# HumanCompatibleAI/overcooked_ai

Measured on NVIDIA H100. Metric: env-steps/sec (joint transitions), higher is better.
Workload: dtype int32

## Files before the change

### overcooked_ai_b200/csrc/ovc_b200.cu

```cuda
#include <cuda.h>
#include <cuda_runtime.h>
#include <stdint.h>
#include <stdio.h>
#include <stdlib.h>
#include <string.h>

#include "../../include/ovc_b200.h"
#include "ovc_step.cuh"

namespace ovc {

static thread_local char g_err[512] = "";

static int fail(int code, const char *msg) {
    snprintf(g_err, sizeof g_err, "%s", msg);
    return code;
}
static int fail(int code, const char *msg, long long value) {
    snprintf(g_err, sizeof g_err, "%s (got %lld)", msg, value);
    return code;
}
static int cuda_fail(cudaError_t e, const char *what) {
    snprintf(g_err, sizeof g_err, "%s: %s", what, cudaGetErrorString(e));
    return OVC_E_CUDA;
}

__device__ __forceinline__ uint32_t smem_u32(const void *p) { return (uint32_t)__cvta_generic_to_shared(p); }

__device__ __forceinline__ void mbar_init(uint64_t *bar, int count) {
    asm volatile("mbarrier.init.shared::cta.b64 [%0], %1;" ::"r"(smem_u32(bar)), "r"(count) : "memory");
    asm volatile("fence.mbarrier_init.release.cluster;" ::: "memory");
    asm volatile("fence.proxy.async.shared::cta;" ::: "memory");
}
__device__ __forceinline__ void mbar_expect_tx(uint64_t *bar, uint32_t bytes) {
    asm volatile("mbarrier.arrive.expect_tx.shared::cta.b64 _, [%0], %1;" ::"r"(smem_u32(bar)), "r"(bytes) : "memory");
}
__device__ __forceinline__ void mbar_wait(uint64_t *bar, uint32_t parity) {
    uint32_t ok;
    do {
        asm volatile(
            "{\n\t.reg .pred p;\n\t"
            "mbarrier.try_wait.parity.shared::cta.b64 p, [%1], %2;\n\t"
            "selp.u32 %0, 1, 0, p;\n\t}"
            : "=r"(ok)
            : "r"(smem_u32(bar)), "r"(parity)
            : "memory");
    } while (!ok);
}
__device__ __forceinline__ void fence_async_smem() { asm volatile("fence.proxy.async.shared::cta;" ::: "memory"); }

__device__ __forceinline__ void tma_load_2d(void *dst, const CUtensorMap *map, int c0, int c1, uint64_t *bar) {
    asm volatile(
        "cp.async.bulk.tensor.2d.shared::cluster.global.tile.mbarrier::complete_tx::bytes [%0], [%1, {%2, %3}], [%4];"
        ::"r"(smem_u32(dst)), "l"((uint64_t)map), "r"(c0), "r"(c1), "r"(smem_u32(bar))
        : "memory");
}
__device__ __forceinline__ void tma_store_2d(const CUtensorMap *map, int c0, int c1, const void *src) {
    asm volatile("cp.async.bulk.tensor.2d.global.shared::cta.tile.bulk_group [%0, {%1, %2}], [%3];" ::"l"((uint64_t)map),
                 "r"(c0), "r"(c1), "r"(smem_u32(src))
                 : "memory");
}
__device__ __forceinline__ void prefetch_tmap(const CUtensorMap *map) {
    asm volatile("prefetch.tensormap [%0];" ::"l"((uint64_t)map) : "memory");
}
__device__ __forceinline__ void prefetch_l2(const void *p) { asm volatile("prefetch.global.L2 [%0];" ::"l"(p)); }
__device__ __forceinline__ void bulk_load_1d(void *dst, const void *src, uint32_t bytes, uint64_t *bar) {
    asm volatile("cp.async.bulk.shared::cluster.global.mbarrier::complete_tx::bytes [%0], [%1], %2, [%3];" ::"r"(
                     smem_u32(dst)),
                 "l"((uint64_t)src), "r"(bytes), "r"(smem_u32(bar))
                 : "memory");
}
__device__ __forceinline__ void bulk_store_1d(void *dst, const void *src, uint32_t bytes) {
    asm volatile("cp.async.bulk.global.shared::cta.bulk_group [%0], [%1], %2;" ::"l"((uint64_t)dst), "r"(smem_u32(src)),
                 "r"(bytes)
                 : "memory");
}
__device__ __forceinline__ void bulk_commit() { asm volatile("cp.async.bulk.commit_group;" ::: "memory"); }
template <int N>
__device__ __forceinline__ void bulk_wait_read() {
    asm volatile("cp.async.bulk.wait_group.read %0;" ::"n"(N) : "memory");
}

template <int S, int SWZ>
struct SmemRec {
    char *tile;
    uint32_t base;
    __device__ __forceinline__ uint32_t phys(uint32_t off) const {
        if (SWZ == 0) return off;
        return off ^ (((off >> 7) & ((1u << SWZ) - 1u)) << 4);
    }
    __device__ __forceinline__ int4 ld4(int c) const { return *reinterpret_cast<const int4 *>(tile + phys(base + c * 16)); }
    __device__ __forceinline__ void st4(int c, int4 v) { *reinterpret_cast<int4 *>(tile + phys(base + c * 16)) = v; }
    __device__ __forceinline__ int ldw(int w) const { return *reinterpret_cast<const int *>(tile + phys(base + w * 4)); }
    __device__ __forceinline__ void stw(int w, int v) { *reinterpret_cast<int *>(tile + phys(base + w * 4)) = v; }
};

struct GlobalRec {
    int32_t *rec;
    __device__ __forceinline__ int4 ld4(int c) const { return *reinterpret_cast<const int4 *>(rec + c * 4); }
    __device__ __forceinline__ void st4(int c, int4 v) { *reinterpret_cast<int4 *>(rec + c * 4) = v; }
    __device__ __forceinline__ int ldw(int w) const { return rec[w]; }
    __device__ __forceinline__ void stw(int w, int v) { rec[w] = v; }
};

#ifndef OVC_TILE16
#define OVC_TILE16 128
#endif

template <int S>
struct Cfg {
    static constexpr int TILE = S <= 16 ? OVC_TILE16 : S <= 32 ? 128 : 64;
    static constexpr int ROW_WORDS = S == 16 ? 16 : 32;
    static constexpr int ROWS_PER_ENV = S / ROW_WORDS;
    static constexpr int BOX_ROWS = TILE * ROWS_PER_ENV;
    static constexpr int SWZ = S == 16 ? 2 : 3;
    static constexpr int TILE_BYTES = TILE * S * 4;
};

struct StepArgs {
    const ovc_layout_t *layouts;
    const int32_t *start_records;
    int32_t *state;
    const int32_t *actions;
    int32_t *sparse, *shaped, *done, *events;
    long long n_envs;
    int n_layouts;
    int n_steps;
    int horizon, flags;
    int has_rs;
    ovc_random_start_t rs;
};

__host__ __device__ __forceinline__ unsigned delivery_rank(unsigned row) { return (unsigned)((0x0008007605432100ull >> (row * 4)) & 15u); }
__host__ __device__ __forceinline__ unsigned delivery_row(unsigned rank) { return (unsigned)((0xC98654321ull >> (rank * 4)) & 15u); }

__device__ __forceinline__ unsigned event_code(unsigned ev) {
    if ((ev & 0x1FFFFFFu) == 0) return 0;
    if (ev & (1u << OVC_EV_SOUP_DELIVERY)) return 23u + delivery_rank((ev >> OVC_EV_RECIPE_SHIFT) & 15u);
    if (ev & ((1u << OVC_EV_POTTING_ONION) | (1u << OVC_EV_POTTING_TOMATO))) {
        const unsigned tom = (ev >> OVC_EV_POTTING_TOMATO) & 1u;
        const unsigned viable = (ev >> (OVC_EV_VIABLE_ONION_POTTING + tom)) & 1u, optimal = (ev >> (OVC_EV_OPTIMAL_ONION_POTTING + tom)) & 1u;
        const unsigned cata = (ev >> (OVC_EV_CATASTROPHIC_ONION_POTTING + tom)) & 1u;
        return 15u + tom * 4u + (viable ? (optimal ? 0u : 1u) : (cata ? 2u : 3u));
    }
    if (ev & (1u << OVC_EV_SOUP_PICKUP)) return 7;
    if (ev & (1u << OVC_EV_SOUP_DROP)) return 14;
    if (ev & (1u << OVC_EV_ONION_PICKUP)) return 1u + ((ev >> OVC_EV_USEFUL_ONION_PICKUP) & 1u);
    if (ev & (1u << OVC_EV_TOMATO_PICKUP)) return 3u + ((ev >> OVC_EV_USEFUL_TOMATO_PICKUP) & 1u);
    if (ev & (1u << OVC_EV_DISH_PICKUP)) return 5u + ((ev >> OVC_EV_USEFUL_DISH_PICKUP) & 1u);
    if (ev & (1u << OVC_EV_ONION_DROP)) return 8u + ((ev >> OVC_EV_USEFUL_ONION_DROP) & 1u);
    if (ev & (1u << OVC_EV_TOMATO_DROP)) return 10u + ((ev >> OVC_EV_USEFUL_TOMATO_DROP) & 1u);
    return 12u + ((ev >> OVC_EV_USEFUL_DISH_DROP) & 1u);
}

__device__ __forceinline__ unsigned code_word(unsigned c0, unsigned c1, unsigned done, bool stepped, bool grant0, bool grant1) {
    return c0 | (c1 << 5) | (done << 10) | (stepped ? 1u << 11 : 0u) | (grant0 ? 1u << 12 : 0u) | (grant1 ? 1u << 13 : 0u);
}

template <bool WIDE>
__device__ __forceinline__ void write_outputs(const StepArgs &a, long long idx, const StepOut &o) {
    if (!WIDE && (a.flags & OVC_F_OUT_CODES)) {
        reinterpret_cast<unsigned short *>(a.events)[idx] = (unsigned short)code_word(
            event_code(o.ev0), event_code(o.ev1), (unsigned)o.done, o.ev0 & OVC_EVF_STEPPED_DONE, o.shaped0 != 0, o.shaped1 != 0);
        return;
    }
    if (!WIDE && (a.flags & OVC_F_OUT_PACKED)) {
        reinterpret_cast<short *>(a.sparse)[idx] = (short)o.sparse;
        reinterpret_cast<char2 *>(a.shaped)[idx] = make_char2((signed char)o.shaped0, (signed char)o.shaped1);
        reinterpret_cast<unsigned short *>(a.events)[idx] = (unsigned short)code_word(
            event_code(o.ev0), event_code(o.ev1), (unsigned)o.done, o.ev0 & OVC_EVF_STEPPED_DONE, false, false);
        return;
    }
    if (!WIDE && (a.flags & OVC_F_OUT_NARROW)) {
        reinterpret_cast<short *>(a.sparse)[idx] = (short)o.sparse;
        reinterpret_cast<unsigned char *>(a.done)[idx] = (unsigned char)o.done;
        reinterpret_cast<char2 *>(a.shaped)[idx] = make_char2((signed char)o.shaped0, (signed char)o.shaped1);
    } else {
        a.sparse[idx] = o.sparse;
        a.done[idx] = o.done;
        reinterpret_cast<int2 *>(a.shaped)[idx] = make_int2(o.shaped0, o.shaped1);
    }
    reinterpret_cast<int2 *>(a.events)[idx] = make_int2((int)o.ev0, (int)o.ev1);
}

template <bool WIDE, typename I>
__device__ __forceinline__ const void *action_addr(const StepArgs &a, I idx) {
    if (!WIDE && (a.flags & OVC_F_ACT_PACKED)) return reinterpret_cast<const unsigned char *>(a.actions) + idx;
    if (!WIDE && (a.flags & OVC_F_ACT_U8)) return reinterpret_cast<const uchar2 *>(a.actions) + idx;
    return reinterpret_cast<const int2 *>(a.actions) + idx;
}

template <bool WIDE, typename I>
__device__ __forceinline__ int2 load_action(const StepArgs &a, I idx) {
    if (!WIDE && (a.flags & OVC_F_ACT_PACKED)) {
        const unsigned u = *static_cast<const unsigned char *>(action_addr<WIDE>(a, idx));
        return make_int2((int)(u & 15u), (int)(u >> 4));
    }
    if (!WIDE && (a.flags & OVC_F_ACT_U8)) {
        const uchar2 u = *static_cast<const uchar2 *>(action_addr<WIDE>(a, idx));
        return make_int2(u.x, u.y);
    }
    return *static_cast<const int2 *>(action_addr<WIDE>(a, idx));
}

constexpr int MAX_SMEM_LAYOUTS = 8;

template <int S, int IO, bool RS, bool WIDE>
__global__ void __launch_bounds__(Cfg<S>::TILE)
step_kernel(const __grid_constant__ CUtensorMap tmap, const StepArgs a) {
    using C = Cfg<S>;
    const long long env0 = (long long)blockIdx.x * C::TILE;
    const long long env = env0 + threadIdx.x;
    const bool live = env < a.n_envs;
    const int T = a.n_steps;

    if (IO == 3) {
        asm volatile("griddepcontrol.launch_dependents;" ::: "memory");
        asm volatile("griddepcontrol.wait;" ::: "memory");
        if (!live) return;
        GlobalRec r{a.state + env * S};
        const TblG tb{reinterpret_cast<const char *>(a.layouts)};
        for (int t = 0; t < T; t++) {
            const long long idx = (long long)t * a.n_envs + env;
            const int2 act = load_action<WIDE>(a, idx);
            StepOut o;
            step_core<RS>(r, tb, a.start_records, S, act.x, act.y, a.horizon, a.flags, RS ? &a.rs : nullptr, env, a.n_layouts, o);
            write_outputs<WIDE>(a, idx, o);
        }
        return;
    }

    extern __shared__ __align__(1024) char smem[];
    char *tile = smem;
    const int n_tbl = a.n_layouts <= MAX_SMEM_LAYOUTS ? a.n_layouts : 0;
    const uint32_t tbl_bytes = (uint32_t)n_tbl * (uint32_t)sizeof(ovc_layout_t);
    char *tbl = smem + C::TILE_BYTES;
    uint64_t *bar = reinterpret_cast<uint64_t *>(smem + C::TILE_BYTES + tbl_bytes);
    const long long rem = a.n_envs - env0;
    const uint32_t live_bytes = (uint32_t)((rem < C::TILE ? rem : C::TILE) * S * 4);

    if (threadIdx.x == 0) {
        mbar_init(bar, 1);
        mbar_expect_tx(bar, (IO == 1 ? (uint32_t)C::TILE_BYTES : live_bytes) + tbl_bytes);
        if (IO == 1) prefetch_tmap(&tmap);
        if (n_tbl) bulk_load_1d(tbl, a.layouts, tbl_bytes, bar);
    }
    asm volatile("griddepcontrol.wait;" ::: "memory");
    if (threadIdx.x == 0) {
        if (IO == 1) tma_load_2d(tile, &tmap, 0, (int)(env0 * C::ROWS_PER_ENV), bar);
        else bulk_load_1d(tile, a.state + env0 * S, live_bytes, bar);
    }
    int2 act = make_int2(OVC_A_STAY, OVC_A_STAY);
    if (live) act = load_action<WIDE>(a, env);
    __syncthreads();
    mbar_wait(bar, 0);
    asm volatile("griddepcontrol.launch_dependents;" ::: "memory");

    if (live) {
        SmemRec<S, IO == 1 ? C::SWZ : 0> r{tile, (uint32_t)threadIdx.x * S * 4};
        auto run = [&](auto tb) {
            for (int t = 0; t < T; t++) {
                const long long idx = (long long)t * a.n_envs + env;
                int2 nxt = act;
                if (t + 1 < T) nxt = load_action<WIDE>(a, idx + a.n_envs);
                StepOut o;
                step_core<RS>(r, tb, a.start_records, S, act.x, act.y, a.horizon, a.flags, RS ? &a.rs : nullptr, env, a.n_layouts, o);
                write_outputs<WIDE>(a, idx, o);
                act = nxt;
            }
        };
        if (n_tbl) run(TblS{tbl});
        else run(TblG{reinterpret_cast<const char *>(a.layouts)});
    }
    fence_async_smem();
    __syncthreads();
    if (threadIdx.x == 0) {
        if (IO == 1) tma_store_2d(&tmap, 0, (int)(env0 * C::ROWS_PER_ENV), tile);
        else bulk_store_1d(a.state + env0 * S, tile, live_bytes);
        bulk_commit();
        bulk_wait_read<0>();
    }
}

}

#include "ovc_rollout.cuh"

namespace ovc {

__global__ void reset_kernel(const int32_t *__restrict__ start_records, int n_layouts, int32_t *__restrict__ state,
                             const int32_t *__restrict__ env_layout, const int32_t *__restrict__ mask,
                             long long n_envs, int S) {
    const int cpr = S / 4;
    const long long i = (long long)blockIdx.x * blockDim.x + threadIdx.x;
    if (i >= n_envs * cpr) return;
    const long long env = i / cpr;
    const int c = (int)(i % cpr);
    if (mask && mask[env] == 0) return;
    int lid = env_layout ? env_layout[env] : (state[env * S + 3] & 0xFF);
    if (lid < 0 || lid >= n_layouts) lid = 0;
    reinterpret_cast<int4 *>(state)[i] = __ldg(reinterpret_cast<const int4 *>(start_records) + (long long)lid * cpr + c);
}

__global__ void reset_random_kernel(const ovc_layout_t *__restrict__ layouts, int n_layouts,
                                    const int32_t *__restrict__ start_records, int32_t *__restrict__ state,
                                    const int32_t *__restrict__ env_layout, const int32_t *__restrict__ mask,
                                    long long n_envs, int S, const ovc_random_start_t rs) {
    const long long env = (long long)blockIdx.x * blockDim.x + threadIdx.x;
    if (env >= n_envs) return;
    if (mask && mask[env] == 0) return;
    int32_t *rec = state + env * S;
    const unsigned old = (unsigned)rec[3];
    int lid = env_layout ? env_layout[env] : (int)(old & 0xFF);
    const unsigned episode = ((old >> 16) + 1u) & 0xFFFFu;
    if (rs.random_layout) lid = random_layout_id(rs, (uint64_t)env, episode, n_layouts);
    if (lid < 0 || lid >= n_layouts) lid = 0;
    const ovc_layout_t *L = layouts + lid;
    random_start_record([&](int w, int32_t v) { rec[w] = v; }, S, start_records + (size_t)lid * S, L->cook_time, L->free_pos,
                        L->n_free, L->n_pots, lid, rs, (uint64_t)env, episode);
}

typedef CUresult (*encode_tiled_fn)(CUtensorMap *, CUtensorMapDataType, cuuint32_t, void *, const cuuint64_t *,
                                    const cuuint64_t *, const cuuint32_t *, const cuuint32_t *, CUtensorMapInterleave,
                                    CUtensorMapSwizzle, CUtensorMapL2promotion, CUtensorMapFloatOOBfill);

static encode_tiled_fn get_encode_fn() {
    static encode_tiled_fn fn = nullptr;
    static bool tried = false;
    if (!tried) {
        tried = true;
        void *p = nullptr;
        cudaDriverEntryPointQueryResult q;
        if (cudaGetDriverEntryPoint("cuTensorMapEncodeTiled", &p, cudaEnableDefault, &q) == cudaSuccess &&
            q == cudaDriverEntryPointSuccess)
            fn = (encode_tiled_fn)p;
    }
    return fn;
}

template <int S>
static int make_tmap(CUtensorMap *m, int32_t *state, long long n_envs, int box_rows = Cfg<S>::BOX_ROWS) {
    using C = Cfg<S>;
    encode_tiled_fn enc = get_encode_fn();
    if (!enc) return fail(OVC_E_CUDA, "cuTensorMapEncodeTiled entry point not available");
    cuuint64_t dims[2] = {(cuuint64_t)C::ROW_WORDS, (cuuint64_t)(n_envs * C::ROWS_PER_ENV)};
    cuuint64_t strides[1] = {(cuuint64_t)C::ROW_WORDS * 4};
    cuuint32_t box[2] = {(cuuint32_t)C::ROW_WORDS, (cuuint32_t)box_rows};
    cuuint32_t estr[2] = {1, 1};
    CUresult r = enc(m, CU_TENSOR_MAP_DATA_TYPE_INT32, 2, state, dims, strides, box, estr, CU_TENSOR_MAP_INTERLEAVE_NONE,
                     S == 16 ? CU_TENSOR_MAP_SWIZZLE_64B : CU_TENSOR_MAP_SWIZZLE_128B, CU_TENSOR_MAP_L2_PROMOTION_NONE,
                     CU_TENSOR_MAP_FLOAT_OOB_FILL_NONE);
    if (r != CUDA_SUCCESS) return fail(OVC_E_CUDA, "cuTensorMapEncodeTiled failed", (long long)r);
    return OVC_OK;
}

struct OutFmt {
    int act, sparse, shaped, done, events;
    bool stream;
    bool missing(const void *act_p, const void *sparse_p, const void *shaped_p, const void *done_p, const void *events_p) const {
        return !act_p || !events_p || (sparse && !sparse_p) || (shaped && !shaped_p) || (done && !stream && !done_p);
    }
    bool wide() const { return act == 8 && sparse == 4; }
};

static OutFmt formats_of(int flags) {
    OutFmt f;
    f.act = (flags & OVC_F_ACT_PACKED) ? 1 : (flags & OVC_F_ACT_U8) ? 2 : 8;
    f.stream = flags & OVC_F_OUT_STREAM;
    if (f.stream) f.sparse = 2, f.shaped = 0, f.done = 2, f.events = 4;
    else if (flags & OVC_F_OUT_CODES) f.sparse = 0, f.shaped = 0, f.done = 0, f.events = 2;
    else if (flags & OVC_F_OUT_PACKED) f.sparse = 2, f.shaped = 2, f.done = 0, f.events = 2;
    else if (flags & OVC_F_OUT_NARROW) f.sparse = 2, f.shaped = 2, f.done = 1, f.events = 8;
    else f.sparse = 4, f.shaped = 8, f.done = 4, f.events = 8;
    return f;
}

template <int S, int IO>
static cudaError_t launch_one(const CUtensorMap &tmap, const StepArgs &a, unsigned grid, size_t smem, cudaStream_t st) {
    using C = Cfg<S>;
    cudaLaunchConfig_t cfg;
    memset(&cfg, 0, sizeof cfg);
    cfg.gridDim = dim3(grid), cfg.blockDim = dim3(C::TILE), cfg.dynamicSmemBytes = smem, cfg.stream = st;
    cudaLaunchAttribute attr[1];
    attr[0].id = cudaLaunchAttributeProgrammaticStreamSerialization;
    attr[0].val.programmaticStreamSerializationAllowed = 1;
    cfg.attrs = attr;
    cfg.numAttrs = (a.flags & OVC_F_PDL) ? 1 : 0;
    const bool wide = formats_of(a.flags).wide();
    if (a.has_rs)
        return wide ? cudaLaunchKernelEx(&cfg, step_kernel<S, IO, true, true>, tmap, a)
                    : cudaLaunchKernelEx(&cfg, step_kernel<S, IO, true, false>, tmap, a);
    return wide ? cudaLaunchKernelEx(&cfg, step_kernel<S, IO, false, true>, tmap, a)
                : cudaLaunchKernelEx(&cfg, step_kernel<S, IO, false, false>, tmap, a);
}

template <int S, int TILE>
static int launch_rollout(const StepArgs &a, cudaStream_t st) {
    using C = RollCfg<S, TILE>;
    CUtensorMap tmap;
    memset(&tmap, 0, sizeof tmap);
    int rc = make_tmap<S>(&tmap, a.state, a.n_envs, C::BOX_ROWS);
    if (rc) return rc;
    const size_t smem = C::smem_bytes(a.n_layouts);
    const OutFmt f = formats_of(a.flags);
    const bool wide = f.wide(), stream = f.stream;
    void (*kern)(const CUtensorMap, const StepArgs) =
        a.has_rs ? (wide ? rollout_kernel<S, TILE, true, FMT_WIDE> : stream ? rollout_kernel<S, TILE, true, FMT_STREAM> : rollout_kernel<S, TILE, true, FMT_HOST>)
                 : (wide ? rollout_kernel<S, TILE, false, FMT_WIDE> : stream ? rollout_kernel<S, TILE, false, FMT_STREAM> : rollout_kernel<S, TILE, false, FMT_HOST>);
    if (smem > 48 * 1024) {
        cudaError_t e = cudaFuncSetAttribute(kern, cudaFuncAttributeMaxDynamicSharedMemorySize, (int)smem);
        if (e != cudaSuccess) return cuda_fail(e, "rollout kernel shared-memory attribute");
    }
    const long long grid = (a.n_envs + TILE - 1) / TILE;
    StepArgs ka = a;
    ka.flags &= ~F_K5_NO_PREFETCH;
#if OVC_K5_PREFETCH > 1
    {
        int dev = 0, n_sm = 0, per_sm = 0;
        cudaError_t e = cudaGetDevice(&dev);
        if (e == cudaSuccess) e = cudaDeviceGetAttribute(&n_sm, cudaDevAttrMultiProcessorCount, dev);
        if (e == cudaSuccess) e = cudaOccupancyMaxActiveBlocksPerMultiprocessor(&per_sm, kern, TILE, smem);
        if (e != cudaSuccess) return cuda_fail(e, "rollout kernel occupancy");
        const long long warps = grid * (TILE / 32);
        if (grid <= (long long)per_sm * n_sm && (warps >= 24LL * n_sm || warps < 12LL * n_sm)) ka.flags |= F_K5_NO_PREFETCH;
    }
#endif
    cudaLaunchConfig_t cfg;
    memset(&cfg, 0, sizeof cfg);
    cfg.gridDim = dim3((unsigned)grid), cfg.blockDim = dim3(TILE), cfg.dynamicSmemBytes = smem, cfg.stream = st;
    cudaLaunchAttribute attr[1];
    attr[0].id = cudaLaunchAttributeProgrammaticStreamSerialization;
    attr[0].val.programmaticStreamSerializationAllowed = 1;
    cfg.attrs = attr;
    cfg.numAttrs = 0;
    cudaError_t e = cudaLaunchKernelEx(&cfg, kern, tmap, ka);
    if (e != cudaSuccess) return cuda_fail(e, "rollout kernel launch");
    return OVC_OK;
}

static int rollout_tile(int S, long long n_envs, int n_layouts) {
    static int forced = -1;
    if (forced < 0) {
        const char *e = getenv("OVC_K5_TILE");
        forced = e ? atoi(e) : 0;
    }
    (void)n_envs;
    if (S > 32) return 64;
    if (forced == 32 || forced == 64 || forced == 128) return forced;
    return n_layouts >= 3 ? 128 : 64;
}

static bool use_rollout_kernel(const StepArgs &a, int io) {
    static int off = -1;
    if (off < 0) {
        const char *e = getenv("OVC_K5_LEGACY");
        off = e && atoi(e) ? 1 : 0;
    }
    const bool stream = a.flags & OVC_F_OUT_STREAM;
    return (!off || stream) && (a.n_steps > 1 || stream) && a.n_steps <= ROLLOUT_MAX_STEPS && io == 1 && a.n_layouts <= MAX_SMEM_LAYOUTS;
}

template <int S>
static int launch_rollout_tiled(const StepArgs &a, cudaStream_t st) {
    if constexpr (S > 32) {
        return launch_rollout<S, 64>(a, st);
    } else {
        switch (rollout_tile(S, a.n_envs, a.n_layouts)) {
        case 32: return launch_rollout<S, 32>(a, st);
        case 64: return launch_rollout<S, 64>(a, st);
        default: return launch_rollout<S, 128>(a, st);
        }
    }
}

template <int S>
static int launch_rollout_any(const StepArgs &a0, cudaStream_t st) {
    long long max_steps = 0xFFFFFFFFLL / a0.n_envs - 1;
    {
        static long long cap = -1;
        if (cap < 0) {
            const char *e = getenv("OVC_K5_MAX_LAUNCH_STEPS");
            cap = e ? atoll(e) : 0;
        }
        if (cap > 0 && cap < max_steps && !(a0.flags & OVC_F_OUT_STREAM)) max_steps = cap;
    }
    if (a0.n_steps <= max_steps) return launch_rollout_tiled<S>(a0, st);
    if (max_steps < 1 || (a0.flags & OVC_F_OUT_STREAM)) return fail(OVC_E_UNSUPPORTED, "rollout too large for one launch (n_steps * n_envs must stay below 2^32)");
    const OutFmt f = formats_of(a0.flags);
    for (long long t0 = 0; t0 < a0.n_steps; t0 += max_steps) {
        StepArgs a = a0;
        const long long off = t0 * a0.n_envs;
        a.n_steps = (int)(a0.n_steps - t0 < max_steps ? a0.n_steps - t0 : max_steps);
        a.actions = reinterpret_cast<const int32_t *>(reinterpret_cast<const char *>(a0.actions) + off * f.act);
        if (a0.sparse) a.sparse = reinterpret_cast<int32_t *>(reinterpret_cast<char *>(a0.sparse) + off * f.sparse);
        if (a0.shaped) a.shaped = reinterpret_cast<int32_t *>(reinterpret_cast<char *>(a0.shaped) + off * f.shaped);
        if (a0.done) a.done = reinterpret_cast<int32_t *>(reinterpret_cast<char *>(a0.done) + off * f.done);
        a.events = reinterpret_cast<int32_t *>(reinterpret_cast<char *>(a0.events) + off * f.events);
        const int rc = launch_rollout_tiled<S>(a, st);
        if (rc) return rc;
    }
    return OVC_OK;
}

template <int S>
static int launch_step(const StepArgs &a, int io, cudaStream_t st) {
    using C = Cfg<S>;
    if (use_rollout_kernel(a, io)) return launch_rollout_any<S>(a, st);
    const unsigned grid = (unsigned)((a.n_envs + C::TILE - 1) / C::TILE);
    CUtensorMap tmap;
    memset(&tmap, 0, sizeof tmap);
    const int n_tbl = a.n_layouts <= MAX_SMEM_LAYOUTS ? a.n_layouts : 0;
    const size_t smem = io == 3 ? 0 : C::TILE_BYTES + (size_t)n_tbl * sizeof(ovc_layout_t) + 16;
    cudaError_t e;
    if (io == 1) {
        int rc = make_tmap<S>(&tmap, a.state, a.n_envs);
        if (rc) return rc;
        e = launch_one<S, 1>(tmap, a, grid, smem, st);
    } else if (io == 2) {
        e = launch_one<S, 2>(tmap, a, grid, smem, st);
    } else {
        e = launch_one<S, 3>(tmap, a, grid, smem, st);
    }
    if (e != cudaSuccess) return cuda_fail(e, "step kernel launch");
    return OVC_OK;
}

static int check_common(const void *layouts, int n_layouts, const void *state, long long n_envs, int S) {
    if (!layouts || !state) return fail(OVC_E_BADARG, "null pointer argument");
    if (n_layouts <= 0 || n_layouts > 256) return fail(OVC_E_BADARG, "n_layouts must be 1..256", (long long)(n_layouts));
    if (n_envs < 0) return fail(OVC_E_BADARG, "negative n_envs");
    if (S != 16 && S != 32 && S != 64 && S != 128)
        return fail(OVC_E_BADARG, "state_words must be 16, 32, 64 or 128", (long long)(S));
    if (((uintptr_t)state & 15) != 0) return fail(OVC_E_BADARG, "state must be 16-byte aligned");
    return OVC_OK;
}

static int step_impl(const void *layouts, int n_layouts, const int32_t *start_records, int32_t *state,
                     const int32_t *actions, int32_t *sparse, int32_t *shaped, int32_t *done, int32_t *events,
                     long long n_envs, int n_steps, int S, int horizon, int flags, const ovc_random_start_t *rs,
                     void *stream) {
    int rc = check_common(layouts, n_layouts, state, n_envs, S);
    if (rc) return rc;
    const OutFmt f = formats_of(flags);
    if (f.stream && (flags & (OVC_F_OUT_CODES | OVC_F_OUT_PACKED | OVC_F_OUT_NARROW)))
        return fail(OVC_E_BADARG, "OVC_F_OUT_STREAM excludes the other output formats");
    if (!start_records || f.missing(actions, sparse, shaped, done, events)) return fail(OVC_E_BADARG, "null pointer argument");
    if (!f.sparse) sparse = nullptr;
    if (!f.shaped) shaped = nullptr;
    if (!f.done) done = nullptr;
    if (f.stream && (((unsigned)flags >> OVC_F_STREAM_CAP_SHIFT) & 0xFFFFu) == 0)
        return fail(OVC_E_BADARG, "OVC_F_OUT_STREAM needs a capacity in flags bits 16-31");
    auto misaligned = [](const void *p, int bytes) { return bytes > 1 && (uintptr_t)p % (uintptr_t)bytes != 0; };
    if (misaligned(actions, f.act) || misaligned(sparse, f.sparse) || misaligned(shaped, f.shaped) || misaligned(done, f.done) ||
        misaligned(events, f.events))
        return fail(OVC_E_BADARG, "actions / sparse / shaped / done / events must be aligned to their element size");
    if (n_steps < 1) return fail(OVC_E_BADARG, "n_steps must be >= 1");
    if (n_envs == 0) return OVC_OK;
    int io = (flags & OVC_F_IO_MASK) >> OVC_F_IO_SHIFT;
    if (io == 0) io = 1;
    if (io < 1 || io > 3) return fail(OVC_E_BADARG, "unknown record I/O strategy", (long long)(io));
    if (io == 1 && (n_envs * (S / (S == 16 ? 16 : 32))) > 0x7FFFFFFFLL) io = 2;
    if (f.stream && (io != 1 || n_layouts > MAX_SMEM_LAYOUTS || n_steps > ROLLOUT_MAX_STEPS))
        return fail(OVC_E_UNSUPPORTED, "OVC_F_OUT_STREAM needs the rollout kernel: default record I/O, at most 8 layouts");
    StepArgs a{(const ovc_layout_t *)layouts, start_records, state, actions, sparse, shaped, done, events,
               n_envs, n_layouts, n_steps, horizon, flags, rs != nullptr, rs ? *rs : ovc_random_start_t{0, 0, 0}};
    cudaStream_t st = (cudaStream_t)stream;
    switch (S) {
    case 16: return launch_step<16>(a, io, st);
    case 32: return launch_step<32>(a, io, st);
    case 64: return launch_step<64>(a, io, st);
    default: return launch_step<128>(a, io, st);
    }
}

}

#include "ovc_obs.cuh"
#include "ovc_encfc.cuh"
#include "ovc_tail.cuh"
#include "ovc_wide.cuh"
#include "ovc_partner.cuh"
#include "ovc_lstm.cuh"
#include "ovc_potential.cuh"
#include "ovc_host.cuh"

extern "C" {

int ovc_abi_version(void) { return OVC_ABI_VERSION; }
size_t ovc_layout_table_size(void) { return sizeof(ovc_layout_t); }
size_t ovc_feat_lut_entry_size(void) { return sizeof(ovc_feat_lut_entry_t); }
const char *ovc_last_error(void) { return ovc::g_err; }

int ovc_step(const void *layouts, int n_layouts, const int32_t *start_records, int32_t *state, const int32_t *actions,
             int32_t *sparse, int32_t *shaped, int32_t *done, int32_t *events, int64_t n_envs, int state_words,
             int horizon, int flags, const ovc_random_start_t *random_start, void *stream) {
    return ovc::step_impl(layouts, n_layouts, start_records, state, actions, sparse, shaped, done, events, n_envs, 1,
                          state_words, horizon, flags, random_start, stream);
}

int ovc_rollout(const void *layouts, int n_layouts, const int32_t *start_records, int32_t *state,
                const int32_t *actions, int32_t *sparse, int32_t *shaped, int32_t *done, int32_t *events,
                int64_t n_envs, int n_steps, int state_words, int horizon, int flags,
                const ovc_random_start_t *random_start, void *stream) {
    return ovc::step_impl(layouts, n_layouts, start_records, state, actions, sparse, shaped, done, events, n_envs,
                          n_steps, state_words, horizon, flags, random_start, stream);
}

int ovc_reset(const void *layouts, int n_layouts, const int32_t *start_records, int32_t *state, const int32_t *env_layout,
              const int32_t *mask, int64_t n_envs, int state_words, const ovc_random_start_t *random_start, void *stream) {
    int rc = ovc::check_common(layouts, n_layouts, state, n_envs, state_words);
    if (rc) return rc;
    if (!start_records) return ovc::fail(OVC_E_BADARG, "null pointer argument");
    if (n_envs == 0) return OVC_OK;
    const int threads = 256;
    if (random_start) {
        ovc::reset_random_kernel<<<(unsigned)((n_envs + threads - 1) / threads), threads, 0, (cudaStream_t)stream>>>(
            (const ovc_layout_t *)layouts, n_layouts, start_records, state, env_layout, mask, n_envs, state_words,
            *random_start);
    } else {
        const long long chunks = (long long)n_envs * (state_words / 4);
        ovc::reset_kernel<<<(unsigned)((chunks + threads - 1) / threads), threads, 0, (cudaStream_t)stream>>>(
            start_records, n_layouts, state, env_layout, mask, n_envs, state_words);
// ... 224 lines not shown
```

### overcooked_ai_b200/csrc/ovc_rollout.cuh

```cuda
#pragma once

#ifndef OVC_K5_PREFETCH
#define OVC_K5_PREFETCH 4
#endif

namespace ovc {

struct Derived {
    uint16_t face[1024];
    uint8_t move[2048];
    int32_t cook5[32];
    int32_t deliver5[32];
    uint8_t potcode5[32][2];
    uint8_t dcode5[32];
    uint8_t pad[32];
};
static_assert(sizeof(Derived) == 4480, "Derived table size");
constexpr int DERIVED_ZERO_CHUNKS = (1024 * 2 + 2048) / 16;
#define OVC_DOFF(field) ((uint32_t)offsetof(Derived, field))
#define OVC_LOFF(field) ((uint32_t)offsetof(ovc_layout_t, field))

constexpr unsigned POT_FROZEN = 1u << 31;
constexpr int ROLLOUT_MAX_STEPS = 1 << 22;

// ... 62 lines not shown
    __device__ __forceinline__ TileRec(uint32_t tile, int tid) {
        rec = tile + (uint32_t)tid * S * 4;
        if (SWZ == 0) xm = 0;
        else if (S <= 32) xm = ((((uint32_t)tid * S * 4) >> 7) & ((1u << SWZ) - 1u)) << 4;
        else xm = (uint32_t)tid * (S / 32);
    }
    __device__ __forceinline__ uint32_t phys(uint32_t off) const {
        if (SWZ == 0) return off;
        if (S <= 32) return off ^ xm;
        return off ^ (((xm + (off >> 7)) & 7u) << 4);
    }
    __device__ __forceinline__ int4 ld4(int c) const { return lds_tile4(rec + phys((uint32_t)c * 16)); }
    __device__ __forceinline__ void st4(int c, int4 v) const { sts_tile4(rec + phys((uint32_t)c * 16), v); }
    __device__ __forceinline__ uint32_t addr(int w) const { return rec + phys((uint32_t)w * 4); }
    __device__ __forceinline__ unsigned ldw(int w) const { return lds_tile(addr(w)); }
    __device__ __forceinline__ void stw(int w, unsigned v) const { sts_tile(addr(w), v); }
};

__device__ __forceinline__ unsigned pot_to_chip(unsigned w, uint32_t D, unsigned clk) {
    const unsigned tp1 = (w >> 8) & 0x3FFFu;
    if ((w & 7u) != OVC_O_SOUP || tp1 == 0) return w & 0x3FFFFFu;
    const unsigned cook = lds_tbl32(D + OVC_DOFF(cook5) + 4u * ((w >> 3) & 31u));
    if (tp1 - 1u > cook) return (w & 0x3FFFFFu) | POT_FROZEN;
    return (w & 0xFFu) | ((clk + (cook - (tp1 - 1u)) + 1u) << 8);
}
__device__ __forceinline__ unsigned pot_to_ext(unsigned w, uint32_t D, unsigned clk) {
    if (w & POT_FROZEN) return w & 0x3FFFFFu;
    const unsigned g = w >> 8;
    if (g == 0) return w;
    const unsigned cook = lds_tbl32(D + OVC_DOFF(cook5) + 4u * ((w >> 3) & 31u));
    const unsigned left = g - 1u > clk ? g - 1u - clk : 0u;
    return (w & 0xFFu) | ((cook - left + 1u) << 8);
}

struct RollOut {
    int sparse, sh0, sh1;
    unsigned c0, c1;
};

constexpr unsigned PS_FULL = 1u, PS_DISH = 1u << 4;
template <class R>
__device__ __forceinline__ unsigned pot_summary(const R &r, int n_pots) {
    unsigned ps = 0;
#pragma unroll 1
    for (int k = 0; k < n_pots; k++) {
        const unsigned w = r.ldw(4 + k);
        const bool soup = (w & 7u) == OVC_O_SOUP;
        const bool idle = (w >> 8) == 0;
        const unsigned n = (w >> 3) & 3u;
        if (soup && (!idle || n == 3u)) ps += PS_FULL;
        if (soup && (!idle || n == 1u || n == 2u)) ps += PS_DISH;
    }
    return ps;
}

template <class R>
__device__ __forceinline__ unsigned interact_v2(const R &r, uint32_t L, uint32_t D, unsigned &me, const unsigned other_t,
                                                unsigned &misc, const unsigned ps, unsigned &psn, const int n_pots,
                                                const bool old_dyn, const unsigned s, int &sparse, int &shaped) {
    const unsigned cell = lds_tbl16(D + OVC_DOFF(face) + 2u * (me & 0x3FFu));
    const unsigned terr = cell & 7u;
    unsigned held = me >> 10;
    const unsigned ht = held & 7u;
    unsigned code = 0;
    if (terr - 1u < 4u) {
        const bool ctr = terr == OVC_T_COUNTER;
        const uint32_t wa = r.addr(4 + (int)(cell >> 8));
        unsigned cw = terr - 1u;
        if (ctr) cw = lds_tile(wa);
        const bool pick = held == 0 && cw != 0;
        const bool drop = ctr && held != 0 && cw == 0;
        if (pick || drop) {
            const unsigned ot = (held | cw) & 7u;
            const unsigned n_full = ps & 15u;
            bool u;
            if (ot == OVC_O_DISH)
                u = pick ? ((misc & 0xFF00u) == 0 && (other_t == OVC_O_DISH ? 1u : 0u) < (ps >> 4)) : (n_full == 0 && other_t != OVC_O_ONION);
            else
                u = ot <= OVC_O_TOMATO && pick != (n_full == (unsigned)n_pots && other_t != OVC_O_DISH);
            code = 2u * ot + (pick ? 0xFFFFFFFFu : 6u) + (unsigned)u;
            if (ctr) {
                sts_tile(wa, held);
                if (ot == OVC_O_DISH) misc += pick ? 0xFFFFFF00u : 0x100u;
            } else {
                if (ot == OVC_O_TOMATO) code = 0;
                if (ot == OVC_O_DISH && u) shaped += (int)lds_tbl32(L + OVC_LOFF(rew_dish_pickup));
            }
            held = pick ? cw : 0u;
        }
    } else if (terr == OVC_T_POT) {
        const uint32_t wa = r.addr(4 + (int)(cell >> 8));
        const unsigned w = lds_tile(wa);
        const unsigned k5 = (w >> 3) & 31u;
        const unsigned n = k5 & 3u;
        if (ht == 0) {
            if (!old_dyn && (w & ~0xF8u) == OVC_O_SOUP && n != 0) {
                sts_tile(wa, w | ((s + lds_tbl32(D + OVC_DOFF(cook5) + 4u * k5) + 1u) << 8));
                psn += n == 3u ? PS_DISH : PS_FULL;
            }
        } else if (ht == OVC_O_DISH) {
            const unsigned g = w >> 8;
            if ((int)w < 0 || g - 1u <= s) {
                code = 7;
                held = pot_to_ext(w, D, s);
                sts_tile(wa, 0u);
                shaped += (int)lds_tbl32(L + OVC_LOFF(rew_soup_pickup));
                psn -= PS_FULL + PS_DISH;
            }
        } else if (ht <= OVC_O_TOMATO) {
            if ((w >> 8) == 0 && n < 3u) {
                const unsigned tom = ht == OVC_O_TOMATO;
                code = lds_tbl8(D + OVC_DOFF(potcode5) + 2u * k5 + tom);
                sts_tile(wa, ((w ? w : (unsigned)OVC_O_SOUP) + 8u) | (tom << (5 + n)));
                shaped += (int)lds_tbl32(L + OVC_LOFF(rew_placement_in_pot));
                held = 0;
                psn += n == 0 ? PS_DISH : n == 2u ? PS_FULL - PS_DISH : 0u;
            }
        }
    } else if (terr == OVC_T_SERVE && ht == OVC_O_SOUP) {
        const unsigned k5 = (held >> 3) & 31u;
        sparse += (int)lds_tbl32(D + OVC_DOFF(deliver5) + 4u * k5);
        code = lds_tbl8(D + OVC_DOFF(dcode5) + k5);
        held = 0;
    }
    me = (me & 0x3FFu) | (held << 10);
    return code;
}

constexpr int FMT_WIDE = 0, FMT_HOST = 1, FMT_STREAM = 2;

constexpr int F_K5_NO_PREFETCH = 1 << 12;

template <int FMT>
struct RollIO {
    static constexpr bool WIDE = FMT == FMT_WIDE;
    const StepArgs &a;
    unsigned oi, ai;
    const unsigned n;
    unsigned live_mask, cnt, cap, lane_lt, mi, n_groups;
    unsigned short *vals;
    bool leader;
    __device__ __forceinline__ RollIO(const StepArgs &args, long long env, unsigned live) : a(args), n((unsigned)args.n_envs) {
        oi = ai = (unsigned)env;
        live_mask = live, cnt = 0, cap = 0, lane_lt = 0, mi = 0, n_groups = 0, vals = nullptr, leader = false;
        if (FMT == FMT_STREAM) {
            n_groups = (unsigned)((a.n_envs + 31) >> 5);
            mi = (unsigned)(env >> 5);
            cap = ((unsigned)a.flags >> OVC_F_STREAM_CAP_SHIFT) & 0xFFFFu;
            const unsigned lane = (unsigned)env & 31u;
            lane_lt = (1u << lane) - 1u, leader = lane == 0;
            vals = reinterpret_cast<unsigned short *>(a.sparse) + (size_t)mi * cap;
        }
    }
    __device__ __forceinline__ int2 load_action() const { return ovc::load_action<WIDE>(a, ai); }
    __device__ __forceinline__ void next_action() { ai += n; }
    __device__ __forceinline__ void prefetch_action(unsigned rows) const { prefetch_l2(action_addr<WIDE>(a, ai + rows * n)); }
    __device__ __forceinline__ void write(const RollOut &o, int done_v, bool stepped, uint32_t mask) {
        const unsigned i = oi;
        oi += n;
        if (FMT == FMT_STREAM) {
            const unsigned w = o.c0 | (o.c1 << 5) | ((unsigned)done_v << 10) | (stepped ? 1u << 11 : 0u) |
                               (o.sh0 != 0 ? 1u << 12 : 0u) | (o.sh1 != 0 ? 1u << 13 : 0u);
            const unsigned m = __ballot_sync(live_mask, w != 0);
            if (leader) reinterpret_cast<unsigned *>(a.events)[mi] = m;
            mi += n_groups;
            if (w != 0) {
                const unsigned pos = cnt + __popc(m & lane_lt);
                if (pos < cap) vals[pos] = (unsigned short)w;
            }
            cnt += __popc(m);
            if (a.done) reinterpret_cast<unsigned short *>(a.done)[i] = (unsigned short)w;
            return;
        }
        if (!WIDE && (a.flags & (OVC_F_OUT_CODES | OVC_F_OUT_PACKED))) {
            unsigned w = o.c0 | (o.c1 << 5) | ((unsigned)done_v << 10) | (stepped ? 1u << 11 : 0u);
            if (a.flags & OVC_F_OUT_CODES) {
                w |= (o.sh0 != 0 ? 1u << 12 : 0u) | (o.sh1 != 0 ? 1u << 13 : 0u);
            } else {
                reinterpret_cast<short *>(a.sparse)[i] = (short)o.sparse;
                reinterpret_cast<char2 *>(a.shaped)[i] = make_char2((signed char)o.sh0, (signed char)o.sh1);
            }
            reinterpret_cast<unsigned short *>(a.events)[i] = (unsigned short)w;
            return;
        }
        const unsigned e0 = stepped ? (unsigned)OVC_EVF_STEPPED_DONE : lds_tbl32(mask + 4u * o.c0);
        const unsigned e1 = stepped ? (unsigned)OVC_EVF_STEPPED_DONE : lds_tbl32(mask + 4u * o.c1);
        if (!WIDE && (a.flags & OVC_F_OUT_NARROW)) {
            reinterpret_cast<short *>(a.sparse)[i] = (short)o.sparse;
            reinterpret_cast<unsigned char *>(a.done)[i] = (unsigned char)done_v;
            reinterpret_cast<char2 *>(a.shaped)[i] = make_char2((signed char)o.sh0, (signed char)o.sh1);
        } else {
            a.sparse[i] = o.sparse;
            a.done[i] = done_v;
            reinterpret_cast<int2 *>(a.shaped)[i] = make_int2(o.sh0, o.sh1);
        }
        reinterpret_cast<int2 *>(a.events)[i] = make_int2((int)e0, (int)e1);
    }
};

template <int S, int TILE>
struct RollCfg {
    static constexpr int ROW_WORDS = S == 16 ? 16 : 32;
    static constexpr int ROWS_PER_ENV = S / ROW_WORDS;
    static constexpr int BOX_ROWS = TILE * ROWS_PER_ENV;
    static constexpr int SWZ = S == 16 ? 2 : 3;
    static constexpr int TILE_BYTES = TILE * S * 4;
    static_assert(BOX_ROWS <= 256, "TMA box rows");
    static_assert(TILE_BYTES % 1024 == 0, "tile must keep the swizzle alignment of what follows");
    static size_t smem_bytes(int n_layouts) { return (size_t)TILE_BYTES + (size_t)n_layouts * (sizeof(ovc_layout_t) + sizeof(Derived)) + 128 + 16; }
};

template <int S, int TILE, bool RS, int FMT>
__global__ void __launch_bounds__(TILE)
rollout_kernel(const __grid_constant__ CUtensorMap tmap, const StepArgs a) {
    using C = RollCfg<S, TILE>;
    constexpr bool WIDE = FMT == FMT_WIDE;
    const int tid = threadIdx.x;
    const long long env0 = (long long)blockIdx.x * TILE;
    const long long env = env0 + tid;
    const bool live = env < a.n_envs;
    const int T = a.n_steps;
    const int n_tbl = a.n_layouts;

    extern __shared__ __align__(1024) char smem[];
    char *tile = smem;
    ovc_layout_t *tbl = reinterpret_cast<ovc_layout_t *>(smem + C::TILE_BYTES);
    Derived *der = reinterpret_cast<Derived *>(smem + C::TILE_BYTES + (size_t)n_tbl * sizeof(ovc_layout_t));
    unsigned *mask = reinterpret_cast<unsigned *>(reinterpret_cast<char *>(der) + (size_t)n_tbl * sizeof(Derived));
    uint64_t *bar = reinterpret_cast<uint64_t *>(mask + 32);
    const uint32_t tbl_bytes = (uint32_t)n_tbl * (uint32_t)sizeof(ovc_layout_t);

    if (tid == 0) {
        mbar_init(bar, 1);
        mbar_expect_tx(bar, (uint32_t)C::TILE_BYTES + tbl_bytes);
        prefetch_tmap(&tmap);
        bulk_load_1d(tbl, a.layouts, tbl_bytes, bar);
    }
    for (int l = 0; l < n_tbl; l++)
        for (int i = tid; i < DERIVED_ZERO_CHUNKS; i += TILE) reinterpret_cast<int4 *>(der + l)[i] = make_int4(0, 0, 0, 0);
    if (tid < 32) mask[tid] = code_mask_of(tid);
    asm volatile("griddepcontrol.wait;" ::: "memory");
    if (tid == 0) tma_load_2d(tile, &tmap, 0, (int)(env0 * C::ROWS_PER_ENV), bar);
    int2 act = make_int2(OVC_A_STAY, OVC_A_STAY);
    if (live) act = load_action<WIDE>(a, env);
#if OVC_K5_PREFETCH > 1
    const bool prefetch = !(a.flags & F_K5_NO_PREFETCH);
    if (live && prefetch)
        for (int k = 1; k < OVC_K5_PREFETCH && k < T; k++) prefetch_l2(action_addr<WIDE>(a, (unsigned)env + (unsigned)k * (unsigned)a.n_envs));
#endif
    __syncthreads();
    mbar_wait(bar, 0);
    asm volatile("griddepcontrol.launch_dependents;" ::: "memory");

    for (int l = 0; l < n_tbl; l++) {
        const ovc_layout_t *L = tbl + l;
        Derived *D = der + l;
        if (tid < 32) {
            const unsigned k5 = tid;
            const int n = k5 & 3, row = recipe_row5(k5);
            D->cook5[k5] = L->cook_time[row];
            D->deliver5[k5] = L->deliver_value[row];
            D->dcode5[k5] = (uint8_t)(23u + delivery_rank((unsigned)row));
            const int old_val = L->best_value[n ? row : 0];
#pragma unroll
            for (int tom = 0; tom < 2; tom++) {
                int cls = 0;
                if (n < 3) {
                    const int new_val = L->best_value[recipe_row5((k5 + 1u) | ((unsigned)tom << (2 + n)))];
                    cls = new_val > 0 ? (old_val == new_val ? 0 : 1) : (old_val > 0 ? 2 : 3);
                }
                D->potcode5[k5][tom] = (uint8_t)(15 + 4 * tom + cls);
            }
        }
        const int n_free = L->n_free;
        for (int i = tid; i < n_free * 12; i += TILE) {
            const int f = i / 12, d = i - f * 12;
            const int pos = L->free_pos[f];
            if (d < 4) {
                D->face[(d << 8) | pos] = L->cell[(pos + dir_delta(d)) & 0xFF];
            } else {
                const int act_i = d - 4;
                int np = pos;
                if (act_i < 4) {
                    const int tp = (pos + dir_delta(act_i)) & 0xFF;
                    if ((L->cell[tp] & 7) == OVC_T_FLOOR) np = tp;
                }
                D->move[(act_i << 8) | pos] = (uint8_t)np;
            }
        }
    }
    __syncthreads();

    const unsigned live_mask = __ballot_sync(0xFFFFFFFFu, live);
    if (live) {
        const TileRec<S, C::SWZ> r(smem_u32(tile), tid);
        const uint32_t tbl_s = smem_u32(tbl), der_s = smem_u32(der), mask_s = smem_u32(mask);
        int t;
        unsigned toff;
        unsigned p0, p1, misc, ps, psn;
        uint32_t L, D;
        int n_pots;
        bool old_dyn;
        auto load_regs = [&](unsigned clk) {
            const int4 h = r.ld4(0);
            t = h.x, p0 = (unsigned)h.y, p1 = (unsigned)h.z, misc = (unsigned)h.w;
            toff = clk - (unsigned)t;
            unsigned lid = misc & 0xFFu;
            if (lid >= (unsigned)n_tbl) lid = 0;
            L = tbl_s + lid * (uint32_t)sizeof(ovc_layout_t), D = der_s + lid * (uint32_t)sizeof(Derived);
            n_pots = (int)lds_tbl32(L + OVC_LOFF(n_pots));
            old_dyn = (lds_tbl32(L + OVC_LOFF(flags)) & OVC_LAYOUT_OLD_DYNAMICS) != 0;
#pragma unroll 1
            for (int k = 0; k < n_pots; k++) r.stw(4 + k, pot_to_chip(r.ldw(4 + k), D, clk));
            ps = psn = pot_summary(r, n_pots);
        };
        load_regs(0u);

        RollIO<FMT> io(a, env, live_mask);

        auto interact = [&](bool second, RollOut &o) {
            unsigned pa = second ? p1 : p0;
            const unsigned pb = second ? p0 : p1;
            int sh = 0;
            const unsigned c = interact_v2(r, L, D, pa, (pb >> 10) & 7u, misc, ps, psn, n_pots, old_dyn, (unsigned)t + toff, o.sparse, sh);
            if (second) p1 = pa, o.sh1 = sh, o.c1 = c;
            else p0 = pa, o.sh0 = sh, o.c0 = c;
        };
        auto finish = [&](int a0, int a1, const RollOut &o, bool stepped) {
            int done = 1;
            if (!stepped) {
                const unsigned o0 = p0 & 0xFFu, o1 = p1 & 0xFFu;
                unsigned n0 = lds_tbl8(D + OVC_DOFF(move) + ((((unsigned)a0 & 7u) << 8) | o0));
                unsigned n1 = lds_tbl8(D + OVC_DOFF(move) + ((((unsigned)a1 & 7u) << 8) | o1));
                const bool collide = n0 == n1 || (n0 == o1 && n1 == o0);
                if (collide) n0 = o0, n1 = o1;
                if ((unsigned)a0 < 4u) p0 = (p0 & ~0x3FFu) | ((unsigned)a0 << 8) | n0;
                if ((unsigned)a1 < 4u) p1 = (p1 & ~0x3FFu) | ((unsigned)a1 << 8) | n1;
                if (old_dyn) {
#pragma unroll 1
                    for (int k = 0; k < n_pots; k++) {
                        const unsigned w = r.ldw(4 + k);
                        if ((w & ~0xE0u) == (OVC_O_SOUP | (3u << 3))) {
                            r.stw(4 + k, w | (((unsigned)t + toff + lds_tbl32(D + OVC_DOFF(cook5) + 4u * ((w >> 3) & 31u)) + 1u) << 8));
                            psn += PS_DISH;
                        }
                    }
                }
                ps = psn;
                done = a.horizon > 0 && t + 1 >= a.horizon;
            }
            io.write(o, done, stepped, mask_s);
            if (stepped) return;
            if (done && (a.flags & OVC_F_AUTO_RESET)) {
                const unsigned lid0 = misc & 0xFFu;
                if (RS && a.has_rs) {
                    const unsigned episode = ((misc >> 16) + 1u) & 0xFFFFu;
                    int lid = (int)lid0;
                    if (a.rs.random_layout) lid = random_layout_id(a.rs, (uint64_t)env, episode, a.n_layouts);
                    const ovc_layout_t *Ln = tbl + lid;
                    random_start_record([&](int w, int32_t v) { r.stw(w, (unsigned)v); }, S, a.start_records + (size_t)lid * S,
                                        Ln->cook_time, Ln->free_pos, Ln->n_free, Ln->n_pots, lid, a.rs, (uint64_t)env, episode);
                } else {
                    const int4 *__restrict__ src = reinterpret_cast<const int4 *>(a.start_records + (size_t)lid0 * S);
#pragma unroll 4
                    for (int c = 0; c < S / 4; c++) r.st4(c, __ldg(src + c));
                }
                load_regs((unsigned)t + toff + 1u);
            } else {
                t = t + 1;
            }
        };

        for (int s = 0; s < T; s++) {
            int2 nxt = act;
            io.next_action();
            if (s + 1 < T) nxt = io.load_action();
#if OVC_K5_PREFETCH > 1
            if (prefetch && s + OVC_K5_PREFETCH < T) io.prefetch_action(OVC_K5_PREFETCH - 1);
#endif
            const int a0 = act.x, a1 = act.y;
            act = nxt;
            RollOut o{0, 0, 0, 0u, 0u};
            bool stepped = a.horizon > 0 && t >= a.horizon;
            if (FMT != FMT_STREAM) {
                if (stepped) {
                    io.write(o, 1, true, mask_s);
                    continue;
                }
                stepped = false;
            }
            if (!stepped) {
                const bool i0 = a0 == OVC_A_INTERACT, i1 = a1 == OVC_A_INTERACT;
                if (i0 || i1) interact(!i0, o);
                if (i0 && i1) interact(true, o);
            }
            finish(a0, a1, o, FMT == FMT_STREAM && stepped);
        }
// ... 15 lines not shown
```

Baseline: 77.50 billion.

## Use streaming cache hints for rollout I/O and 32-thread tiles when grid fits

Rollout action loads now use __ldcs and output stores use __stcs streaming hints. The L2 prefetch of future actions gets an evict_last policy. When the 64-env tile would be chosen and no tile is forced, the launcher checks occupancy and switches to 32-thread blocks if the whole grid fits in one wave. The goal is less cache pollution from write-once outputs and more SMs busy at small env counts. The cost is an extra occupancy query on every launch and possible cache-policy interactions that hurt reuse.

```diff
diff --git a/overcooked_ai_b200/csrc/ovc_b200.cu b/overcooked_ai_b200/csrc/ovc_b200.cu
--- a/overcooked_ai_b200/csrc/ovc_b200.cu
+++ b/overcooked_ai_b200/csrc/ovc_b200.cu
@@ -63,7 +63,7 @@
 __device__ __forceinline__ void prefetch_tmap(const CUtensorMap *map) {
     asm volatile("prefetch.tensormap [%0];" ::"l"((uint64_t)map) : "memory");
 }
-__device__ __forceinline__ void prefetch_l2(const void *p) { asm volatile("prefetch.global.L2 [%0];" ::"l"(p)); }
+__device__ __forceinline__ void prefetch_l2(const void *p) { asm volatile("prefetch.global.L2::evict_last [%0];" ::"l"(p)); }
 __device__ __forceinline__ void bulk_load_1d(void *dst, const void *src, uint32_t bytes, uint64_t *bar) {
     asm volatile("cp.async.bulk.shared::cluster.global.mbarrier::complete_tx::bytes [%0], [%1], %2, [%3];" ::"r"(
                      smem_u32(dst)),
@@ -201,6 +201,19 @@
         return make_int2(u.x, u.y);
     }
     return *static_cast<const int2 *>(action_addr<WIDE>(a, idx));
+}
+
+template <bool WIDE, typename I>
+__device__ __forceinline__ int2 load_action_last(const StepArgs &a, I idx) {
+    if (!WIDE && (a.flags & OVC_F_ACT_PACKED)) {
+        const unsigned u = __ldcs(static_cast<const unsigned char *>(action_addr<WIDE>(a, idx)));
+        return make_int2((int)(u & 15u), (int)(u >> 4));
+    }
+    if (!WIDE && (a.flags & OVC_F_ACT_U8)) {
+        const uchar2 u = __ldcs(static_cast<const uchar2 *>(action_addr<WIDE>(a, idx)));
+        return make_int2(u.x, u.y);
+    }
+    return __ldcs(static_cast<const int2 *>(action_addr<WIDE>(a, idx)));
 }
 
 constexpr int MAX_SMEM_LAYOUTS = 8;
@@ -394,6 +407,16 @@
                 : cudaLaunchKernelEx(&cfg, step_kernel<S, IO, false, false>, tmap, a);
 }
 
+typedef void (*rollout_fn)(const CUtensorMap, const StepArgs);
+
+template <int S, int TILE>
+static rollout_fn rollout_kernel_for(const StepArgs &a) {
+    const OutFmt f = formats_of(a.flags);
+    const bool wide = f.wide(), stream = f.stream;
+    return a.has_rs ? (wide ? rollout_kernel<S, TILE, true, FMT_WIDE> : stream ? rollout_kernel<S, TILE, true, FMT_STREAM> : rollout_kernel<S, TILE, true, FMT_HOST>)
+                    : (wide ? rollout_kernel<S, TILE, false, FMT_WIDE> : stream ? rollout_kernel<S, TILE, false, FMT_STREAM> : rollout_kernel<S, TILE, false, FMT_HOST>);
+}
+
 template <int S, int TILE>
 static int launch_rollout(const StepArgs &a, cudaStream_t st) {
     using C = RollCfg<S, TILE>;
@@ -402,11 +425,7 @@
     int rc = make_tmap<S>(&tmap, a.state, a.n_envs, C::BOX_ROWS);
     if (rc) return rc;
     const size_t smem = C::smem_bytes(a.n_layouts);
-    const OutFmt f = formats_of(a.flags);
-    const bool wide = f.wide(), stream = f.stream;
-    void (*kern)(const CUtensorMap, const StepArgs) =
-        a.has_rs ? (wide ? rollout_kernel<S, TILE, true, FMT_WIDE> : stream ? rollout_kernel<S, TILE, true, FMT_STREAM> : rollout_kernel<S, TILE, true, FMT_HOST>)
-                 : (wide ? rollout_kernel<S, TILE, false, FMT_WIDE> : stream ? rollout_kernel<S, TILE, false, FMT_STREAM> : rollout_kernel<S, TILE, false, FMT_HOST>);
+    const rollout_fn kern = rollout_kernel_for<S, TILE>(a);
     if (smem > 48 * 1024) {
         cudaError_t e = cudaFuncSetAttribute(kern, cudaFuncAttributeMaxDynamicSharedMemorySize, (int)smem);
         if (e != cudaSuccess) return cuda_fail(e, "rollout kernel shared-memory attribute");
@@ -438,16 +457,27 @@
     return OVC_OK;
 }
 
-static int rollout_tile(int S, long long n_envs, int n_layouts) {
+static int rollout_tile_forced() {
     static int forced = -1;
     if (forced < 0) {
         const char *e = getenv("OVC_K5_TILE");
         forced = e ? atoi(e) : 0;
     }
-    (void)n_envs;
+    return forced == 32 || forced == 64 || forced == 128 ? forced : 0;
+}
+static int rollout_tile(int S, int n_layouts) {
     if (S > 32) return 64;
-    if (forced == 32 || forced == 64 || forced == 128) return forced;
+    if (rollout_tile_forced()) return rollout_tile_forced();
     return n_layouts >= 3 ? 128 : 64;
+}
+
+template <int S>
+static bool one_warp_grid_fits_one_wave(const StepArgs &a) {
+    int dev = 0, n_sm = 0, per_sm = 0;
+    if (cudaGetDevice(&dev) != cudaSuccess || cudaDeviceGetAttribute(&n_sm, cudaDevAttrMultiProcessorCount, dev) != cudaSuccess ||
+        cudaOccupancyMaxActiveBlocksPerMultiprocessor(&per_sm, rollout_kernel_for<S, 32>(a), 32, RollCfg<S, 32>::smem_bytes(a.n_layouts)) != cudaSuccess)
+        return false;
+    return (a.n_envs + 31) / 32 <= (long long)per_sm * n_sm;
 }
 
 static bool use_rollout_kernel(const StepArgs &a, int io) {
@@ -465,9 +495,9 @@
     if constexpr (S > 32) {
         return launch_rollout<S, 64>(a, st);
     } else {
-        switch (rollout_tile(S, a.n_envs, a.n_layouts)) {
+        switch (rollout_tile(S, a.n_layouts)) {
         case 32: return launch_rollout<S, 32>(a, st);
-        case 64: return launch_rollout<S, 64>(a, st);
+        case 64: return !rollout_tile_forced() && one_warp_grid_fits_one_wave<S>(a) ? launch_rollout<S, 32>(a, st) : launch_rollout<S, 64>(a, st);
         default: return launch_rollout<S, 128>(a, st);
         }
     }
diff --git a/overcooked_ai_b200/csrc/ovc_rollout.cuh b/overcooked_ai_b200/csrc/ovc_rollout.cuh
--- a/overcooked_ai_b200/csrc/ovc_rollout.cuh
+++ b/overcooked_ai_b200/csrc/ovc_rollout.cuh
@@ -238,7 +238,7 @@
             vals = reinterpret_cast<unsigned short *>(a.sparse) + (size_t)mi * cap;
         }
     }
-    __device__ __forceinline__ int2 load_action() const { return ovc::load_action<WIDE>(a, ai); }
+    __device__ __forceinline__ int2 load_action() const { return load_action_last<WIDE>(a, ai); }
     __device__ __forceinline__ void next_action() { ai += n; }
     __device__ __forceinline__ void prefetch_action(unsigned rows) const { prefetch_l2(action_addr<WIDE>(a, ai + rows * n)); }
     __device__ __forceinline__ void write(const RollOut &o, int done_v, bool stepped, uint32_t mask) {
@@ -248,14 +248,14 @@
             const unsigned w = o.c0 | (o.c1 << 5) | ((unsigned)done_v << 10) | (stepped ? 1u << 11 : 0u) |
                                (o.sh0 != 0 ? 1u << 12 : 0u) | (o.sh1 != 0 ? 1u << 13 : 0u);
             const unsigned m = __ballot_sync(live_mask, w != 0);
-            if (leader) reinterpret_cast<unsigned *>(a.events)[mi] = m;
+            if (leader) __stcs(reinterpret_cast<unsigned *>(a.events) + mi, m);
             mi += n_groups;
             if (w != 0) {
                 const unsigned pos = cnt + __popc(m & lane_lt);
-                if (pos < cap) vals[pos] = (unsigned short)w;
+                if (pos < cap) __stcs(vals + pos, (unsigned short)w);
             }
             cnt += __popc(m);
-            if (a.done) reinterpret_cast<unsigned short *>(a.done)[i] = (unsigned short)w;
+            if (a.done) __stcs(reinterpret_cast<unsigned short *>(a.done) + i, (unsigned short)w);
             return;
         }
         if (!WIDE && (a.flags & (OVC_F_OUT_CODES | OVC_F_OUT_PACKED))) {
@@ -263,24 +263,24 @@
             if (a.flags & OVC_F_OUT_CODES) {
                 w |= (o.sh0 != 0 ? 1u << 12 : 0u) | (o.sh1 != 0 ? 1u << 13 : 0u);
             } else {
-                reinterpret_cast<short *>(a.sparse)[i] = (short)o.sparse;
-                reinterpret_cast<char2 *>(a.shaped)[i] = make_char2((signed char)o.sh0, (signed char)o.sh1);
-            }
-            reinterpret_cast<unsigned short *>(a.events)[i] = (unsigned short)w;
+                __stcs(reinterpret_cast<short *>(a.sparse) + i, (short)o.sparse);
+                __stcs(reinterpret_cast<char2 *>(a.shaped) + i, make_char2((signed char)o.sh0, (signed char)o.sh1));
+            }
+            __stcs(reinterpret_cast<unsigned short *>(a.events) + i, (unsigned short)w);
             return;
         }
         const unsigned e0 = stepped ? (unsigned)OVC_EVF_STEPPED_DONE : lds_tbl32(mask + 4u * o.c0);
         const unsigned e1 = stepped ? (unsigned)OVC_EVF_STEPPED_DONE : lds_tbl32(mask + 4u * o.c1);
         if (!WIDE && (a.flags & OVC_F_OUT_NARROW)) {
-            reinterpret_cast<short *>(a.sparse)[i] = (short)o.sparse;
-            reinterpret_cast<unsigned char *>(a.done)[i] = (unsigned char)done_v;
-            reinterpret_cast<char2 *>(a.shaped)[i] = make_char2((signed char)o.sh0, (signed char)o.sh1);
+            __stcs(reinterpret_cast<short *>(a.sparse) + i, (short)o.sparse);
+            __stcs(reinterpret_cast<unsigned char *>(a.done) + i, (unsigned char)done_v);
+            __stcs(reinterpret_cast<char2 *>(a.shaped) + i, make_char2((signed char)o.sh0, (signed char)o.sh1));
         } else {
-            a.sparse[i] = o.sparse;
-            a.done[i] = done_v;
-            reinterpret_cast<int2 *>(a.shaped)[i] = make_int2(o.sh0, o.sh1);
-        }
-        reinterpret_cast<int2 *>(a.events)[i] = make_int2((int)e0, (int)e1);
+            __stcs(a.sparse + i, o.sparse);
+            __stcs(a.done + i, done_v);
+            __stcs(reinterpret_cast<int2 *>(a.shaped) + i, make_int2(o.sh0, o.sh1));
+        }
+        __stcs(reinterpret_cast<int2 *>(a.events) + i, make_int2((int)e0, (int)e1));
     }
 };
 
@@ -328,7 +328,7 @@
     asm volatile("griddepcontrol.wait;" ::: "memory");
     if (tid == 0) tma_load_2d(tile, &tmap, 0, (int)(env0 * C::ROWS_PER_ENV), bar);
     int2 act = make_int2(OVC_A_STAY, OVC_A_STAY);
-    if (live) act = load_action<WIDE>(a, env);
+    if (live) act = load_action_last<WIDE>(a, env);
 #if OVC_K5_PREFETCH > 1
     const bool prefetch = !(a.flags & F_K5_NO_PREFETCH);
     if (live && prefetch)
```

Result: faster. 79.48 billion (median of 6 runs) (+2.6%).
